# stevewongv/Sparse2Dense

Measured on AMD Instinct MI355X. Metric: LiDAR frames/sec (fwd+bwd), 150k-pt 0.1m-voxel synthetic Waymo scene, higher is better.
Workload: dtype bf16 (sparse stack: bf16 storage; dense neck/head: bf16 NHWC activations; fp32 accumulate, statistics, master weights, optimizer)

## Files before the change

### include/s2d.h

```cpp
#ifndef S2D_H_
#define S2D_H_

#include <stddef.h>
#include <stdint.h>

#ifdef __cplusplus
extern "C" {
#endif

typedef void *s2d_stream_t;

#define S2D_OK 0
#define S2D_ERR_INVALID_ARG (-1)
#define S2D_ERR_UNSUPPORTED (-2)
#define S2D_ERR_CAPACITY (-3)
#define S2D_ERR_WORKSPACE (-4)
#define S2D_ERR_COMM (-5)

int s2d_version(void);
int s2d_last_error(char *buf, size_t buf_len);
int s2d_build_info(char *buf, size_t buf_len);

size_t s2d_voxelize_batch_workspace_bytes(int frames, const int64_t *point_offsets, int max_points, int max_voxels);
int s2d_voxelize_batch_run(const float *points, int frames, const int64_t *point_offsets, int ndim,
                           const float coors_range[6], const float voxel_size[3], int max_points, int max_voxels,
                           float *voxels, int32_t *coors4, int32_t *num_points, float *mean, int32_t *out_m,
                           int32_t *out_base, void *ws, size_t ws_bytes, s2d_stream_t stream);
size_t s2d_voxelize_workspace_bytes(int64_t n_points, int max_points, int max_voxels);
int s2d_voxelize_run(const float *points, int64_t n_points, int ndim, const float coors_range[6],
                     const float voxel_size[3], int max_points, int max_voxels, float *voxels,
                     int32_t *coors, int32_t *num_points, float *mean, int32_t *out_m, void *ws,
                     size_t ws_bytes, s2d_stream_t stream);

size_t s2d_rulebook_workspace_bytes(int batch, const int32_t shape[3], int64_t n_rows);

int s2d_rulebook_subm_build(const int32_t *coors, int64_t n, int batch, const int32_t shape[3],
                            const int32_t ksize[3], const int32_t dilation[3], int32_t *nbr_out,
                            int32_t *pair_count, void *ws, size_t ws_bytes, s2d_stream_t stream);

int s2d_rulebook_conv_count(const int32_t *coors, int64_t n, int batch, const int32_t shape[3],
                            const int32_t ksize[3], const int32_t stride[3],
                            const int32_t padding[3], const int32_t dilation[3], int32_t *out_n,
                            void *ws, size_t ws_bytes, s2d_stream_t stream);
int s2d_rulebook_conv_fill(const int32_t *coors, int64_t n, int batch, const int32_t shape[3],
                           const int32_t ksize[3], const int32_t stride[3],
                           const int32_t padding[3], const int32_t dilation[3], int64_t n_out,
                           int32_t *out_coors, int32_t *nbr_out, int32_t *nbr_in,
                           int32_t *pair_count, void *ws, size_t ws_bytes, s2d_stream_t stream);

int s2d_rulebook_chain_supported(int batch, const int32_t shape0[3], int n_strided, const int32_t *ksize,
                                 const int32_t *stride, const int32_t *padding);
size_t s2d_rulebook_chain_workspace_bytes(int batch, const int32_t shape0[3], int n_strided, const int32_t *ksize,
                                          const int32_t *stride, const int32_t *padding);
int s2d_rulebook_chain_plan(const int32_t *coors0, int64_t n0, int batch, const int32_t shape0[3], int n_strided,
                            const int32_t *ksize, const int32_t *stride, const int32_t *padding, int32_t *counts,
                            void *ws, size_t ws_bytes, s2d_stream_t stream);
int s2d_rulebook_chain_fill(const int32_t *coors0, int64_t n0, int batch, const int32_t shape0[3], int n_strided,
                            const int32_t *ksize, const int32_t *stride, const int32_t *padding, const int64_t *n_rows,
                            int32_t *const *out_coors, int32_t *const *subm_nbr, int32_t *const *conv_nbr_out,
                            int32_t *const *conv_nbr_in, int32_t *pair_counts, int32_t *child, void *ws, size_t ws_bytes,
                            s2d_stream_t stream);

int s2d_spconv_fwd_f32(const float *in_feat, int64_t n_in, const float *weight, const float *bias,
                       const int32_t *nbr, int64_t n_out, int kvol, int cin, int cout,
                       float *out_feat, s2d_stream_t stream);
int s2d_spconv_bf16_supported(int cin, int cout);
int s2d_spconv_pack_weights_bf16(const float *weight, int kvol, int cin, int cout, int transpose,
                                 int flip, void *packed, s2d_stream_t stream);
int s2d_spconv_fwd_bf16(const float *in_feat, int64_t n_in, const void *packed_weight,
                        const float *bias, const int32_t *nbr, int64_t n_out, int kvol, int cin,
                        int cout, float *out_feat, s2d_stream_t stream);
size_t s2d_spconv_wgrad_workspace_bytes(int64_t n_out, int kvol, int cin, int cout);
int s2d_spconv_wgrad_f32(const float *in_feat, int64_t n_in, const float *dout, const int32_t *nbr,
                         int64_t n_out, int kvol, int cin, int cout, float *dweight, void *ws,
                         size_t ws_bytes, s2d_stream_t stream);

int s2d_spconv_wgrad_bf16(const float *in_feat, int64_t n_in, const float *dout, const int32_t *nbr,
                          int64_t n_out, int kvol, int cin, int cout, float *dweight, void *ws,
                          size_t ws_bytes, s2d_stream_t stream);

size_t s2d_bn1d_workspace_bytes(int64_t n, int c);
int s2d_bn1d_stats_f32(const float *x, int64_t n, int c, float *stats, void *ws, size_t ws_bytes,
                       s2d_stream_t stream);
int s2d_bn1d_finalize_fwd_f32(const float *stats, const float *count, const float *gamma,
                              const float *beta, float eps, float momentum, int c, float *mean,
                              float *invstd, float *scale, float *shift, float *running_mean,
                              float *running_var, int64_t *batches_tracked, s2d_stream_t stream);
int s2d_bn1d_finalize_bwd_f32(const float *sums_local, const float *sums_global, const float *count,
                              const float *gamma, const float *mean, const float *invstd, int c,
                              float *dgamma, float *dbeta, float *a, float *b, float *d,
                              s2d_stream_t stream);
int s2d_bn1d_stats_finalize_f32(const float *x, int64_t n, int c, const float *gamma,
                                const float *beta, float eps, float momentum, float *mean,
                                float *invstd, float *scale, float *shift, float *running_mean,
                                float *running_var, int64_t *batches_tracked, void *ws,
                                size_t ws_bytes, s2d_stream_t stream);
int s2d_bn1d_bwd_reduce_finalize_f32(const float *dy, const float *y, const float *x, int relu,
                                     int64_t n, int c, const float *gamma, const float *mean,
                                     const float *invstd, float *g_out, float *dgamma, float *dbeta,
                                     float *a, float *b, float *d, void *ws, size_t ws_bytes,
                                     s2d_stream_t stream);
int s2d_bn1d_apply_f32(const float *x, const float *scale, const float *shift,
                       const float *residual, int relu, int64_t n, int c, float *y,
                       s2d_stream_t stream);
int s2d_bn1d_bwd_reduce_f32(const float *dy, const float *y, const float *x, int relu, int64_t n,
                            int c, float *g_out, float *sums, void *ws, size_t ws_bytes,
                            s2d_stream_t stream);
int s2d_bn1d_bwd_apply_f32(const float *g, const float *x, const float *a, const float *b,
                           const float *d, int64_t n, int c, float *dx, s2d_stream_t stream);

// ... 424 lines not shown
```

### sparse2dense_amd/_lib.py

```python
import ctypes
import os

_HERE = os.path.dirname(os.path.abspath(__file__))
LIB_PATH = os.path.join(_HERE, "lib", "libs2d_hip.so")

c_i32p = ctypes.c_void_p
c_f32p = ctypes.c_void_p
_I3 = ctypes.c_int32 * 3
_PFN_GEO = [ctypes.c_int64, ctypes.c_int, ctypes.c_int, ctypes.c_float, ctypes.c_float, ctypes.c_float, ctypes.c_float]
_F3 = ctypes.c_float * 3
_F6 = ctypes.c_float * 6

SIGNATURES = {
    "s2d_version": (ctypes.c_int, []),
    "s2d_last_error": (ctypes.c_int, [ctypes.c_char_p, ctypes.c_size_t]),
    "s2d_build_info": (ctypes.c_int, [ctypes.c_char_p, ctypes.c_size_t]),
    "s2d_debug_lds_fill": (ctypes.c_int, [ctypes.c_float, ctypes.c_int, ctypes.c_int, ctypes.c_void_p, ctypes.c_void_p]),
    "s2d_voxelize_workspace_bytes": (ctypes.c_size_t, [ctypes.c_int64, ctypes.c_int, ctypes.c_int]),
    "s2d_voxelize_run": (ctypes.c_int, [c_f32p, ctypes.c_int64, ctypes.c_int, _F6, _F3, ctypes.c_int, ctypes.c_int,
                                        c_f32p, c_i32p, c_i32p, c_f32p, c_i32p, ctypes.c_void_p, ctypes.c_size_t,
                                        ctypes.c_void_p]),
    "s2d_voxelize_batch_workspace_bytes": (ctypes.c_size_t, [ctypes.c_int, ctypes.c_void_p, ctypes.c_int, ctypes.c_int]),
    "s2d_voxelize_batch_run": (ctypes.c_int, [c_f32p, ctypes.c_int, ctypes.c_void_p, ctypes.c_int, _F6, _F3, ctypes.c_int, ctypes.c_int,
                                              c_f32p, c_i32p, c_i32p, c_f32p, c_i32p, c_i32p, ctypes.c_void_p, ctypes.c_size_t, ctypes.c_void_p]),
    "s2d_rulebook_workspace_bytes": (ctypes.c_size_t, [ctypes.c_int, _I3, ctypes.c_int64]),
    "s2d_rulebook_subm_build": (ctypes.c_int, [c_i32p, ctypes.c_int64, ctypes.c_int, _I3, _I3, _I3, c_i32p, c_i32p,
                                               ctypes.c_void_p, ctypes.c_size_t, ctypes.c_void_p]),
    "s2d_rulebook_conv_count": (ctypes.c_int, [c_i32p, ctypes.c_int64, ctypes.c_int, _I3, _I3, _I3, _I3, _I3, c_i32p,
                                               ctypes.c_void_p, ctypes.c_size_t, ctypes.c_void_p]),
    "s2d_rulebook_conv_fill": (ctypes.c_int, [c_i32p, ctypes.c_int64, ctypes.c_int, _I3, _I3, _I3, _I3, _I3,
                                              ctypes.c_int64, c_i32p, c_i32p, c_i32p, c_i32p, ctypes.c_void_p,
                                              ctypes.c_size_t, ctypes.c_void_p]),
    "s2d_conv2d_pack_batch_bf16": (ctypes.c_int, [ctypes.c_int] + [ctypes.c_void_p] * 9),
    "s2d_pfn_supported": (ctypes.c_int, [ctypes.c_int] * 4),
    "s2d_pfn_blocks": (ctypes.c_int, [ctypes.c_int64]),
    "s2d_pfn_bwd_cols": (ctypes.c_int, []),
    "s2d_pfn_stats_f32": (ctypes.c_int, [c_f32p, c_i32p, c_i32p, c_f32p, ctypes.c_int64, ctypes.c_int, ctypes.c_int, ctypes.c_float, ctypes.c_float,
                                         ctypes.c_float, ctypes.c_float, c_f32p, ctypes.c_void_p]),
    "s2d_pfn_apply_max_f32": (ctypes.c_int, [c_f32p, c_i32p, c_i32p, c_f32p, c_f32p, c_f32p, ctypes.c_int64, ctypes.c_int, ctypes.c_int, ctypes.c_float,
                                             ctypes.c_float, ctypes.c_float, ctypes.c_float, c_f32p, ctypes.c_void_p, ctypes.c_void_p]),
    "s2d_pfn_bwd_f32": (ctypes.c_int, [c_f32p, c_i32p, c_i32p, c_f32p, c_f32p, ctypes.c_void_p, ctypes.c_int64, ctypes.c_int, ctypes.c_int, ctypes.c_float,
                                       ctypes.c_float, ctypes.c_float, ctypes.c_float, c_f32p, ctypes.c_void_p]),
    "s2d_pfn2_supported": (ctypes.c_int, [ctypes.c_int] * 5),
    "s2d_pfn2_bwd_rows": (ctypes.c_int, []),
    "s2d_pfn2_bwd_cols": (ctypes.c_int, []),
    "s2d_pfn2_stats1_f32": (ctypes.c_int, [c_f32p, c_i32p, c_i32p, c_f32p] + _PFN_GEO + [c_f32p, ctypes.c_void_p]),
    "s2d_pfn2_stats2_f32": (ctypes.c_int, [c_f32p, c_i32p, c_i32p, c_f32p, c_f32p, c_f32p] + _PFN_GEO + [c_f32p, ctypes.c_void_p]),
    "s2d_pfn2_apply_max_f32": (ctypes.c_int, [c_f32p, c_i32p, c_i32p, c_f32p, c_f32p, c_f32p, c_f32p] + _PFN_GEO
                               + [c_f32p, ctypes.c_void_p, c_f32p, ctypes.c_void_p]),
    "s2d_pfn2_bwd_f32": (ctypes.c_int, [c_f32p, c_i32p, c_i32p, c_f32p, c_f32p, c_f32p, c_f32p, c_f32p, ctypes.c_void_p] + _PFN_GEO
                         + [c_f32p, ctypes.c_void_p]),
    "s2d_rulebook_chain_supported": (ctypes.c_int, [ctypes.c_int, _I3, ctypes.c_int, ctypes.c_void_p, ctypes.c_void_p, ctypes.c_void_p]),
    "s2d_rulebook_chain_workspace_bytes": (ctypes.c_size_t, [ctypes.c_int, _I3, ctypes.c_int, ctypes.c_void_p, ctypes.c_void_p,
                                                             ctypes.c_void_p]),
    "s2d_rulebook_chain_plan": (ctypes.c_int, [c_i32p, ctypes.c_int64, ctypes.c_int, _I3, ctypes.c_int, ctypes.c_void_p, ctypes.c_void_p,
                                               ctypes.c_void_p, c_i32p, ctypes.c_void_p, ctypes.c_size_t, ctypes.c_void_p]),
    "s2d_rulebook_chain_fill": (ctypes.c_int, [c_i32p, ctypes.c_int64, ctypes.c_int, _I3, ctypes.c_int, ctypes.c_void_p, ctypes.c_void_p,
                                               ctypes.c_void_p, ctypes.c_void_p, ctypes.c_void_p, ctypes.c_void_p, ctypes.c_void_p,
                                               ctypes.c_void_p, c_i32p, c_i32p, ctypes.c_void_p, ctypes.c_size_t, ctypes.c_void_p]),
    "s2d_spconv_fwd_f32": (ctypes.c_int, [c_f32p, ctypes.c_int64, c_f32p, c_f32p, c_i32p, ctypes.c_int64, ctypes.c_int,
                                          ctypes.c_int, ctypes.c_int, c_f32p, ctypes.c_void_p]),
    "s2d_spconv_bf16_supported": (ctypes.c_int, [ctypes.c_int, ctypes.c_int]),
    "s2d_spconv_pack_weights_bf16": (ctypes.c_int, [c_f32p, ctypes.c_int, ctypes.c_int, ctypes.c_int, ctypes.c_int,
                                                    ctypes.c_int, ctypes.c_void_p, ctypes.c_void_p]),
    "s2d_spconv_fwd_bf16": (ctypes.c_int, [c_f32p, ctypes.c_int64, ctypes.c_void_p, c_f32p, c_i32p, ctypes.c_int64,
                                           ctypes.c_int, ctypes.c_int, ctypes.c_int, c_f32p, ctypes.c_void_p]),
    "s2d_spconv_wgrad_workspace_bytes": (ctypes.c_size_t, [ctypes.c_int64, ctypes.c_int, ctypes.c_int, ctypes.c_int]),
    "s2d_spconv_wgrad_f32": (ctypes.c_int, [c_f32p, ctypes.c_int64, c_f32p, c_i32p, ctypes.c_int64, ctypes.c_int,
                                            ctypes.c_int, ctypes.c_int, c_f32p, ctypes.c_void_p, ctypes.c_size_t,
                                            ctypes.c_void_p]),
    "s2d_spconv_wgrad_bf16": (ctypes.c_int, [c_f32p, ctypes.c_int64, c_f32p, c_i32p, ctypes.c_int64, ctypes.c_int,
                                             ctypes.c_int, ctypes.c_int, c_f32p, ctypes.c_void_p, ctypes.c_size_t,
                                             ctypes.c_void_p]),
    "s2d_bn1d_workspace_bytes": (ctypes.c_size_t, [ctypes.c_int64, ctypes.c_int]),
    "s2d_bn1d_stats_f32": (ctypes.c_int, [c_f32p, ctypes.c_int64, ctypes.c_int, c_f32p, ctypes.c_void_p,
                                          ctypes.c_size_t, ctypes.c_void_p]),
    "s2d_bn1d_finalize_fwd_f32": (ctypes.c_int, [c_f32p, c_f32p, c_f32p, c_f32p, ctypes.c_float, ctypes.c_float, ctypes.c_int,
                                                 c_f32p, c_f32p, c_f32p, c_f32p, c_f32p, c_f32p, ctypes.c_void_p,
                                                 ctypes.c_void_p]),
    "s2d_bn1d_finalize_bwd_f32": (ctypes.c_int, [c_f32p, c_f32p, c_f32p, c_f32p, c_f32p, c_f32p, ctypes.c_int, c_f32p,
                                                 c_f32p, c_f32p, c_f32p, c_f32p, ctypes.c_void_p]),
    "s2d_bn1d_stats_finalize_f32": (ctypes.c_int, [c_f32p, ctypes.c_int64, ctypes.c_int, c_f32p, c_f32p, ctypes.c_float,
                                                   ctypes.c_float, c_f32p, c_f32p, c_f32p, c_f32p, c_f32p, c_f32p,
                                                   ctypes.c_void_p, ctypes.c_void_p, ctypes.c_size_t, ctypes.c_void_p]),
    "s2d_bn1d_bwd_reduce_finalize_f32": (ctypes.c_int, [c_f32p, c_f32p, c_f32p, ctypes.c_int, ctypes.c_int64, ctypes.c_int,
                                                        c_f32p, c_f32p, c_f32p, c_f32p, c_f32p, c_f32p, c_f32p, c_f32p,
                                                        c_f32p, ctypes.c_void_p, ctypes.c_size_t, ctypes.c_void_p]),
    "s2d_bn1d_apply_f32": (ctypes.c_int, [c_f32p, c_f32p, c_f32p, c_f32p, ctypes.c_int, ctypes.c_int64, ctypes.c_int,
                                          c_f32p, ctypes.c_void_p]),
    "s2d_bn1d_bwd_reduce_f32": (ctypes.c_int, [c_f32p, c_f32p, c_f32p, ctypes.c_int, ctypes.c_int64, ctypes.c_int,
                                               c_f32p, c_f32p, ctypes.c_void_p, ctypes.c_size_t, ctypes.c_void_p]),
    "s2d_bn1d_bwd_apply_f32": (ctypes.c_int, [c_f32p, c_f32p, c_f32p, c_f32p, c_f32p, ctypes.c_int64, ctypes.c_int,
                                              c_f32p, ctypes.c_void_p]),
    "s2d_pointwise_conv_f32": (ctypes.c_int, [c_f32p, c_f32p, c_f32p, ctypes.c_int, ctypes.c_int, ctypes.c_int,
                                              ctypes.c_int64, c_f32p, ctypes.c_void_p]),
    "s2d_comm_load_library": (ctypes.c_int, [ctypes.c_char_p]),
    "s2d_comm_available": (ctypes.c_int, []),
    "s2d_comm_unique_id": (ctypes.c_int, [ctypes.c_void_p]),
    "s2d_comm_init": (ctypes.c_int, [ctypes.c_void_p, ctypes.c_int, ctypes.c_int]),
    "s2d_comm_ranks": (ctypes.c_int, []),
    "s2d_comm_shutdown": (ctypes.c_int, []),
    "s2d_convt3d_mfma_supported": (ctypes.c_int, [ctypes.c_int, ctypes.c_int]),
    "s2d_convt3d_mfma_packed_elems": (ctypes.c_size_t, [ctypes.c_int, ctypes.c_int]),
    "s2d_convt3d_mfma_pack_weights": (ctypes.c_int, [c_f32p, ctypes.c_int, ctypes.c_int, ctypes.c_void_p, ctypes.c_void_p]),
    "s2d_convt3d_mfma_fwd": (ctypes.c_int, [c_f32p, ctypes.c_void_p, c_f32p] + [ctypes.c_int] * 6 + [c_f32p, ctypes.c_void_p]),
    "s2d_convt3d_mfma_stats_tiles": (ctypes.c_int64, [ctypes.c_int] * 5),
    "s2d_convt3d_mfma_fwd_stats": (ctypes.c_int, [c_f32p, ctypes.c_void_p, c_f32p] + [ctypes.c_int] * 6 + [c_f32p, c_f32p, ctypes.c_void_p]),
# ... 343 lines not shown
```

### sparse2dense_amd/csrc/voxelize.hip

```cpp
#include <limits.h>

#include "s2d_common.h"
#include "scan.h"

namespace s2d {

constexpr uint32_t VOX_EMPTY = 0x7F7F7F7Fu;
constexpr int IDX_EMPTY = 0x7F7F7F7F;

struct VoxParams {
    float lo[3];
    float vs[3];
    int grid[3];
    int ndim;
    int max_points;
    int max_voxels;
    uint32_t table_mask;
    int table_shift;
};

__device__ __forceinline__ uint32_t vox_hash(uint32_t key, int shift) { return (key * 2654435761u) >> shift; }

__device__ __forceinline__ uint32_t vox_table_insert(uint32_t *__restrict__ keys, int *__restrict__ first, uint32_t key, uint32_t h, uint32_t mask, int i) {
    while (true) {
// ... 545 lines not shown
}

extern "C" size_t s2d_voxelize_batch_workspace_bytes(int frames, const int64_t *point_offsets, int max_points, int max_voxels) {
    if (frames <= 0 || frames > VOXB_MAX_FRAMES || !point_offsets || max_points <= 0 || max_voxels <= 0) return 0;
    return voxb_carve(nullptr, frames, point_offsets, max_points, max_voxels).bytes;
}

extern "C" int s2d_voxelize_batch_run(const float *points, int frames, const int64_t *point_offsets, int ndim, const float coors_range[6],
                                      const float voxel_size[3], int max_points, int max_voxels, float *voxels, int32_t *coors4,
                                      int32_t *num_points, float *mean, int32_t *out_m, int32_t *out_base, void *ws, size_t ws_bytes,
                                      s2d_stream_t stream) {
    S2D_CHECK_ARG(frames > 0 && frames <= VOXB_MAX_FRAMES && point_offsets, "voxelize_batch: 1..%d frames", VOXB_MAX_FRAMES);
    S2D_CHECK_ARG(ndim >= 3 && max_points > 0 && max_voxels > 0, "voxelize_batch: bad ndim/max_points/max_voxels");
    S2D_CHECK_ARG(coors_range && voxel_size && out_m && out_base && coors4 && voxels && num_points, "voxelize_batch: null argument");
    const int64_t n_points = point_offsets[frames];
    S2D_CHECK_ARG(point_offsets[0] == 0 && n_points >= 0 && n_points < (int64_t)INT_MAX / 2, "voxelize_batch: bad offsets");
    S2D_CHECK_ARG(n_points == 0 || points, "voxelize_batch: null points");
    hipStream_t st = (hipStream_t)stream;
    VoxParams p;
    double cells = 1.0;
    for (int j = 0; j < 3; ++j) {
        p.lo[j] = coors_range[j];
        p.vs[j] = voxel_size[j];
        float g = (coors_range[3 + j] - coors_range[j]) / voxel_size[j];
        p.grid[j] = (int)nearbyintf(g);
        S2D_CHECK_ARG(p.grid[j] > 0, "voxelize_batch: empty grid on axis %d", j);
        cells *= p.grid[j];
    }
    if (cells >= (double)VOX_EMPTY) {
        set_error("voxelize_batch: grid of %.0f cells exceeds the key space", cells);
        return S2D_ERR_UNSUPPORTED;
    }
    p.ndim = ndim; p.max_points = max_points; p.max_voxels = max_voxels; p.table_mask = 0; p.table_shift = 0;
    VoxbWs w = voxb_carve(ws, frames, point_offsets, max_points, max_voxels);
    if (ws_bytes < w.bytes || !ws) {
        set_error("voxelize_batch: workspace too small (%zu < %zu)", ws_bytes, w.bytes);
        return S2D_ERR_WORKSPACE;
    }
    VoxBatch vb;
    vb.frames = frames;
    int64_t rows = 0;
    size_t tb = 0;
    for (int b = 0; b < frames; ++b) {
        S2D_CHECK_ARG(point_offsets[b + 1] >= point_offsets[b], "voxelize_batch: offsets must not decrease");
        const int64_t nb = point_offsets[b + 1] - point_offsets[b];
        const size_t t = voxb_table(nb);
        int lg = 0;
        while (((size_t)1 << lg) < t) ++lg;
        vb.offs[b] = (int)point_offsets[b];
        vb.table_base[b] = (int)tb;
        vb.table_mask[b] = (uint32_t)(t - 1);
        vb.table_shift[b] = 32 - lg;
        tb += t;
        rows += nb < max_voxels ? nb : max_voxels;
    }
    vb.offs[frames] = (int)n_points;
    if (n_points == 0) {
        S2D_HIP(hipMemsetAsync(out_m, 0, sizeof(int32_t) * frames, st));
        S2D_HIP(hipMemsetAsync(out_base, 0, sizeof(int32_t) * (frames + 1), st));
        return S2D_OK;
    }
    const int n = (int)n_points;
    S2D_HIP(hipMemsetAsync(w.keys, 0x7F, w.clear_bytes, st));
    const dim3 blk(256);
    hipLaunchKernelGGL(voxb_insert_kernel, dim3((n + 255) / 256), blk, 0, st, points, n, p, vb, w.keys, w.first, w.pt_slot, w.total + 1);
    S2D_LAUNCH_CHECK();
    FirstFlagIn fin{w.pt_slot, w.first};
    VoxbRankOut fout{w.pt_slot, w.rank_of_slot, w.frame_start_rank, vb, n};
    int rc = device_exclusive_scan_onepass(fin, fout, n_points, w.flags, w.total, w.total + 1, st);
    if (rc) return rc;
    hipLaunchKernelGGL(voxb_frame_counts_kernel, dim3(1), dim3(64), 0, st, w.frame_start_rank, vb, max_voxels, out_m, w.out_base, out_base, w.total + 1);
    hipLaunchKernelGGL(voxb_assign_kernel, dim3((n + 255) / 256), blk, 0, st, w.pt_slot, w.first, w.keys, w.rank_of_slot, w.frame_start_rank,
                       w.out_base, n, p, vb, w.vid, coors4);
    rc = vox_select_launch(w.pt_slot, w.first, w.vid, n, max_points, rows, w.ksmall, w.sel, st);
    if (rc) return rc;
    hipLaunchKernelGGL(voxb_fill_kernel, dim3((unsigned)ceil_div(rows * max_points, 256)), blk, 0, st, points, w.ksmall, w.out_base, frames, ndim,
                       max_points, voxels, num_points);
    if (mean)
        hipLaunchKernelGGL(voxb_mean_kernel, dim3((unsigned)ceil_div(rows * ndim, 256)), blk, 0, st, points, w.ksmall, w.out_base, frames, ndim,
                           max_points, mean);
    S2D_LAUNCH_CHECK();
    return S2D_OK;
}
```

### sparse2dense_amd/hip_ops.py

```python
import ctypes
import os
from dataclasses import dataclass
from typing import Optional, Tuple

import numpy as np
import torch

from . import _lib
from ._lib import check, f3, f6, i3


def _stream():
    return torch._C._cuda_getCurrentRawStream(torch.cuda.current_device())


def _ptr(t: Optional[torch.Tensor]):
    if t is None:
        return None
    return t.data_ptr()


def _need_gpu(*ts):
    for t in ts:
        if t is not None and not t.is_cuda:
            raise _lib.S2DError("sparse2dense_amd HIP op called with a CPU tensor: there is no CPU fallback")


def _ws(nbytes, device):
    return torch.empty(max(int(nbytes), 256), dtype=torch.uint8, device=device)


def _ws_shared(nbytes, device):
    from .dense2d import _ws as shared_ws
    return shared_ws(nbytes, device)


def voxelize_async(points: torch.Tensor, voxel_size, coors_range, max_points: int, max_voxels: int, with_mean=True):
    lib = _lib.load()
    _need_gpu(points)
    points = points.contiguous().float()
    n, ndim = points.shape
    dev = points.device
    rows = max(min(n, max_voxels), 1)
    voxels = torch.empty((rows, max_points, ndim), dtype=torch.float32, device=dev)
    coors = torch.empty((rows, 3), dtype=torch.int32, device=dev)
    num = torch.empty((rows,), dtype=torch.int32, device=dev)
    mean = torch.empty((rows, ndim), dtype=torch.float32, device=dev) if with_mean else None
    out_m = torch.zeros((1,), dtype=torch.int32, device=dev)
    ws = _ws(lib.s2d_voxelize_workspace_bytes(n, max_points, max_voxels), dev)
    check(lib.s2d_voxelize_run(_ptr(points), n, ndim, f6(coors_range), f3(voxel_size), max_points, max_voxels,
                               _ptr(voxels), _ptr(coors), _ptr(num), _ptr(mean), _ptr(out_m), _ptr(ws), ws.numel(),
                               _stream()), "s2d_voxelize_run")
    return voxels, coors, num, mean, out_m


def voxelize(points: torch.Tensor, voxel_size, coors_range, max_points: int, max_voxels: int, with_mean=True):
    voxels, coors, num, mean, out_m = voxelize_async(points, voxel_size, coors_range, max_points, max_voxels, with_mean)
    m = int(out_m.item())
    if m < 0:
        raise _lib.S2DError("s2d_voxelize_run: the look-back scan timed out on the device (csrc/scan.h); no voxels were produced")
    return voxels[:m], coors[:m], num[:m], (mean[:m] if with_mean else None)


def voxelize_batch_launch(points_cat: torch.Tensor, offsets, voxel_size, coors_range, max_points: int, max_voxels: int):
    lib = _lib.load()
    _need_gpu(points_cat)
    points_cat = points_cat.contiguous().float()
    n, ndim = points_cat.shape
    frames = len(offsets) - 1
    assert offsets[0] == 0 and offsets[-1] == n
    offs = (ctypes.c_int64 * (frames + 1))(*[int(o) for o in offsets])
    dev = points_cat.device
    rows = max(sum(min(int(offsets[b + 1] - offsets[b]), max_voxels) for b in range(frames)), 1)
    voxels = torch.empty((rows, max_points, ndim), dtype=torch.float32, device=dev)
    coors = torch.empty((rows, 4), dtype=torch.int32, device=dev)
    num = torch.empty((rows,), dtype=torch.int32, device=dev)
    mean = torch.empty((rows, ndim), dtype=torch.float32, device=dev)
    out_m = torch.empty((frames,), dtype=torch.int32, device=dev)
    out_base = torch.empty((frames + 1,), dtype=torch.int32, device=dev)
    ws = _ws(lib.s2d_voxelize_batch_workspace_bytes(frames, offs, max_points, max_voxels), dev)
    rec = None
    if PROFILE is not None:
        rec = dict(kernel="voxelize", tag="voxelize", cin=0, cout=0, n_points=int(n), frames=frames, out_base=out_base, max_points=max_points,
                   ndim=int(ndim), start=torch.cuda.Event(enable_timing=True), end=torch.cuda.Event(enable_timing=True))
        rec["start"].record()
    check(lib.s2d_voxelize_batch_run(_ptr(points_cat), frames, offs, ndim, f6(coors_range), f3(voxel_size), max_points, max_voxels,
                                     _ptr(voxels), _ptr(coors), _ptr(num), _ptr(mean), _ptr(out_m), _ptr(out_base), _ptr(ws), ws.numel(),
                                     _stream()), "s2d_voxelize_batch_run")
    if rec is not None:
        rec["end"].record()
        PROFILE.append(rec)
    return (voxels, coors, num, mean, out_base)


def voxelize_batch_collect(pending, base):
    voxels, coors, num, mean, out_base = pending
    m = int(base[-1])
    if m < 0:
        raise _lib.S2DError("s2d_voxelize_batch_run: the look-back scan timed out on the device (csrc/scan.h); no voxels were produced")
    counts = torch.tensor([int(base[b + 1]) - int(base[b]) for b in range(len(base) - 1)], dtype=torch.int64, device=voxels.device)
    return voxels[:m], coors[:m], num[:m], mean[:m], counts


def voxelize_batch(points_cat: torch.Tensor, offsets, voxel_size, coors_range, max_points: int, max_voxels: int):
    pending = voxelize_batch_launch(points_cat, offsets, voxel_size, coors_range, max_points, max_voxels)
    return voxelize_batch_collect(pending, pending[4].cpu().tolist())


@dataclass
class Rulebook:
    subm: bool
    kvol: int
    n_in: int
    n_out: int
    nbr_out: torch.Tensor
    nbr_in: Optional[torch.Tensor]
    pair_count: torch.Tensor
    out_coors: Optional[torch.Tensor]
    out_shape: Tuple[int, int, int]
    coors: Optional[torch.Tensor] = None

    def pairs(self):
        nb = self.nbr_out.cpu().numpy()
        res = []
        for k in range(self.kvol):
            o = np.nonzero(nb[k] >= 0)[0]
            res.append((nb[k][o].astype(np.int64), o.astype(np.int64)))
        return res


def conv_out_shape(shape, ksize, stride, padding, dilation=(1, 1, 1)):
    return tuple((int(shape[i]) + 2 * padding[i] - dilation[i] * (ksize[i] - 1) - 1) // stride[i] + 1 for i in range(3))


def build_subm_rulebook(coors: torch.Tensor, batch: int, shape, ksize, dilation=(1, 1, 1)) -> Rulebook:
    lib = _lib.load()
    _need_gpu(coors)
    coors = coors.contiguous()
    assert coors.dtype == torch.int32 and coors.dim() == 2 and coors.shape[1] == 4
    n = coors.shape[0]
    dev = coors.device
    kvol = int(ksize[0] * ksize[1] * ksize[2])
    nbr = torch.empty((kvol, n), dtype=torch.int32, device=dev)
    cnt = torch.empty((kvol,), dtype=torch.int32, device=dev)
    ws = _ws(lib.s2d_rulebook_workspace_bytes(batch, i3(shape), n), dev)
    rec = None
    if PROFILE is not None:
        rec = dict(kernel="rulebook_subm", tag="rulebook", cin=0, cout=0, n_out=int(n), kvol=kvol, pairs=cnt,
                   start=torch.cuda.Event(enable_timing=True), end=torch.cuda.Event(enable_timing=True))
        rec["start"].record()
    check(lib.s2d_rulebook_subm_build(_ptr(coors), n, batch, i3(shape), i3(ksize), i3(dilation), _ptr(nbr), _ptr(cnt),
                                      _ptr(ws), ws.numel(), _stream()), "s2d_rulebook_subm_build")
    if rec is not None:
        rec["end"].record()
        PROFILE.append(rec)
    return Rulebook(True, kvol, n, n, nbr, None, cnt, None, tuple(int(s) for s in shape), coors=coors)


class ConvRulebookJob:

    def __init__(self, coors, batch, shape, ksize, stride, padding, dilation=(1, 1, 1)):
        self.lib = _lib.load()
        _need_gpu(coors)
        self.coors = coors.contiguous()
        assert self.coors.dtype == torch.int32 and self.coors.shape[1] == 4
        self.batch, self.shape = int(batch), tuple(int(s) for s in shape)
        self.ksize, self.stride = tuple(map(int, ksize)), tuple(map(int, stride))
        self.padding, self.dilation = tuple(map(int, padding)), tuple(map(int, dilation))
        self.out_shape = conv_out_shape(self.shape, self.ksize, self.stride, self.padding, self.dilation)
        self.kvol = self.ksize[0] * self.ksize[1] * self.ksize[2]
        dev = self.coors.device
        self.ws = _ws(self.lib.s2d_rulebook_workspace_bytes(self.batch, i3(self.out_shape), 0), dev)
        self.out_n = torch.zeros((1,), dtype=torch.int32, device=dev)

    def count(self):
        n = self.coors.shape[0]
        self._rec = None
        if PROFILE is not None:
            self._rec = dict(kernel="rulebook_conv", tag="rulebook", cin=0, cout=0, n_in=int(n), kvol=self.kvol,
                             start=torch.cuda.Event(enable_timing=True), end=torch.cuda.Event(enable_timing=True),
                             start2=torch.cuda.Event(enable_timing=True), end2=torch.cuda.Event(enable_timing=True))
            self._rec["start"].record()
        check(self.lib.s2d_rulebook_conv_count(_ptr(self.coors), n, self.batch, i3(self.shape), i3(self.ksize),
                                               i3(self.stride), i3(self.padding), i3(self.dilation), _ptr(self.out_n),
                                               _ptr(self.ws), self.ws.numel(), _stream()), "s2d_rulebook_conv_count")
        if self._rec is not None:
            self._rec["end"].record()
        return self

# ... 484 lines not shown
```

### sparse2dense_amd/voxel_ops.py

```python
import numpy as np
import torch

from . import hip_ops as H


def points_to_voxel(points, voxel_size, coors_range, max_points=35, reverse_index=True, max_voxels=20000,
                    return_mean=False):
    is_np = isinstance(points, np.ndarray)
    if is_np:
        if not torch.cuda.is_available():
            raise RuntimeError("points_to_voxel: no ROCm device visible and there is no CPU fallback")
        pts = torch.from_numpy(np.ascontiguousarray(points, dtype=np.float32)).cuda()
    else:
        pts = points
    vs = np.asarray(voxel_size, dtype=np.float32)
    rng = np.asarray(coors_range, dtype=np.float32)
    voxels, coors, num, mean = H.voxelize(pts, vs, rng, int(max_points), int(max_voxels), with_mean=return_mean)
    if not reverse_index:
        coors = coors.flip(1)
    if is_np:
        out = (voxels.cpu().numpy(), coors.cpu().numpy(), num.cpu().numpy())
        return out + (mean.cpu().numpy(),) if return_mean else out
    return (voxels, coors, num, mean) if return_mean else (voxels, coors, num)


class VoxelGenerator:
    def __init__(self, voxel_size, point_cloud_range, max_num_points, max_voxels=20000):
        point_cloud_range = np.array(point_cloud_range, dtype=np.float32)
        voxel_size = np.array(voxel_size, dtype=np.float32)
        grid_size = (point_cloud_range[3:] - point_cloud_range[:3]) / voxel_size
        self._grid_size = np.round(grid_size).astype(np.int64)
        self._voxel_size = voxel_size
        self._point_cloud_range = point_cloud_range
        self._max_num_points = max_num_points
        self._max_voxels = max_voxels

    def generate(self, points, max_voxels=-1, return_mean=False):
        if max_voxels == -1:
            max_voxels = self._max_voxels
        return points_to_voxel(points, self._voxel_size, self._point_cloud_range, self._max_num_points, True,
                               max_voxels, return_mean=return_mean)

    @property
    def voxel_size(self):
        return self._voxel_size

    @property
    def max_num_points_per_voxel(self):
        return self._max_num_points

    @property
    def point_cloud_range(self):
        return self._point_cloud_range

    @property
    def grid_size(self):
        return self._grid_size


def voxelize_batches(requests):
    pend = []
    for generator, point_clouds, prefix in requests:
        offs = [0]
        for pts in point_clouds:
            offs.append(offs[-1] + int(pts.shape[0]))
        cat = point_clouds[0] if len(point_clouds) == 1 else torch.cat([p.float() for p in point_clouds], 0)
        pend.append((prefix, H.voxelize_batch_launch(cat, offs, generator.voxel_size, generator.point_cloud_range,
                                                     generator.max_num_points_per_voxel, generator._max_voxels)))
    bases = torch.cat([p[1][4] for p in pend]).cpu().tolist()
    out, at = {}, 0
    for prefix, p in pend:
        k = p[4].numel()
        v, c, n, m, counts = H.voxelize_batch_collect(p, bases[at:at + k])
        at += k
        out.update({prefix + "voxels": v, prefix + "coordinates": c, prefix + "num_points": n, prefix + "num_voxels": counts,
                    prefix + "voxel_mean": m})
    return out


def voxelize_batch(generator: VoxelGenerator, point_clouds, max_voxels=-1, prefix="", batched=True):
    mv = generator._max_voxels if max_voxels == -1 else max_voxels
    if batched and point_clouds[0].is_cuda and len(point_clouds) <= 64:
        offs = [0]
        for pts in point_clouds:
            offs.append(offs[-1] + int(pts.shape[0]))
        cat = point_clouds[0] if len(point_clouds) == 1 else torch.cat([p.float() for p in point_clouds], 0)
        v, c, n, m, counts = H.voxelize_batch(cat, offs, generator.voxel_size, generator.point_cloud_range,
                                              generator.max_num_points_per_voxel, mv)
        return {prefix + "voxels": v, prefix + "coordinates": c, prefix + "num_points": n, prefix + "num_voxels": counts,
                prefix + "voxel_mean": m}
    pend = [H.voxelize_async(pts, generator.voxel_size, generator.point_cloud_range, generator.max_num_points_per_voxel,
                             generator._max_voxels if max_voxels == -1 else max_voxels, with_mean=True)
            for pts in point_clouds]
    counts = torch.cat([p[4] for p in pend]).cpu().tolist()
    if counts and min(counts) < 0:
        raise H._lib.S2DError("s2d_voxelize_run: the look-back scan timed out on the device (csrc/scan.h)")
    vs, cs, ns, ms = [], [], [], []
    for b, ((v, c, n, m, _), k) in enumerate(zip(pend, counts)):
        cb = torch.empty((k, 4), dtype=torch.int32, device=c.device)
        cb[:, 0] = b
        cb[:, 1:] = c[:k]
        vs.append(v[:k]); cs.append(cb); ns.append(n[:k]); ms.append(m[:k])
    dev = vs[0].device
    return {
        prefix + "voxels": torch.cat(vs, 0),
        prefix + "coordinates": torch.cat(cs, 0),
        prefix + "num_points": torch.cat(ns, 0),
        prefix + "num_voxels": torch.tensor(counts, dtype=torch.int64, device=dev),
        prefix + "voxel_mean": torch.cat(ms, 0),
    }
```

Baseline: 225.7.

## Voxelize all segments in one radix-sort based multi-segment launch

Measured after the change: 228.7 (median of 5 runs). 1.4% higher.

```diff
diff --git a/include/s2d.h b/include/s2d.h
--- a/include/s2d.h
+++ b/include/s2d.h
@@ -26,6 +26,21 @@
                            const float coors_range[6], const float voxel_size[3], int max_points, int max_voxels,
                            float *voxels, int32_t *coors4, int32_t *num_points, float *mean, int32_t *out_m,
                            int32_t *out_base, void *ws, size_t ws_bytes, s2d_stream_t stream);
+typedef struct s2d_vox_segment {
+    float coors_range[6];
+    float voxel_size[3];
+    int32_t max_points, max_voxels, ndim, frames;
+    const float *const *frame_points;
+    const int64_t *frame_counts;
+    float *voxels;
+    int32_t *coors4;
+    int32_t *num_points;
+    float *mean;
+    int32_t *out_m;
+} s2d_vox_segment;
+size_t s2d_voxelize_multi_workspace_bytes(int segments, const s2d_vox_segment *segs);
+int s2d_voxelize_multi_run(int segments, const s2d_vox_segment *segs, int32_t *out_base_all, void *ws, size_t ws_bytes,
+                           s2d_stream_t stream);
 size_t s2d_voxelize_workspace_bytes(int64_t n_points, int max_points, int max_voxels);
 int s2d_voxelize_run(const float *points, int64_t n_points, int ndim, const float coors_range[6],
                      const float voxel_size[3], int max_points, int max_voxels, float *voxels,
diff --git a/sparse2dense_amd/_lib.py b/sparse2dense_amd/_lib.py
--- a/sparse2dense_amd/_lib.py
+++ b/sparse2dense_amd/_lib.py
@@ -10,6 +10,15 @@
 _PFN_GEO = [ctypes.c_int64, ctypes.c_int, ctypes.c_int, ctypes.c_float, ctypes.c_float, ctypes.c_float, ctypes.c_float]
 _F3 = ctypes.c_float * 3
 _F6 = ctypes.c_float * 6
+
+
+
+class VoxSegment(ctypes.Structure):
+    _fields_ = [("coors_range", _F6), ("voxel_size", _F3), ("max_points", ctypes.c_int32), ("max_voxels", ctypes.c_int32),
+                ("ndim", ctypes.c_int32), ("frames", ctypes.c_int32), ("frame_points", ctypes.c_void_p), ("frame_counts", ctypes.c_void_p),
+                ("voxels", ctypes.c_void_p), ("coors4", ctypes.c_void_p), ("num_points", ctypes.c_void_p), ("mean", ctypes.c_void_p),
+                ("out_m", ctypes.c_void_p)]
+
 
 SIGNATURES = {
     "s2d_version": (ctypes.c_int, []),
@@ -23,6 +32,8 @@
     "s2d_voxelize_batch_workspace_bytes": (ctypes.c_size_t, [ctypes.c_int, ctypes.c_void_p, ctypes.c_int, ctypes.c_int]),
     "s2d_voxelize_batch_run": (ctypes.c_int, [c_f32p, ctypes.c_int, ctypes.c_void_p, ctypes.c_int, _F6, _F3, ctypes.c_int, ctypes.c_int,
                                               c_f32p, c_i32p, c_i32p, c_f32p, c_i32p, c_i32p, ctypes.c_void_p, ctypes.c_size_t, ctypes.c_void_p]),
+    "s2d_voxelize_multi_workspace_bytes": (ctypes.c_size_t, [ctypes.c_int, ctypes.c_void_p]),
+    "s2d_voxelize_multi_run": (ctypes.c_int, [ctypes.c_int, ctypes.c_void_p, c_i32p, ctypes.c_void_p, ctypes.c_size_t, ctypes.c_void_p]),
     "s2d_rulebook_workspace_bytes": (ctypes.c_size_t, [ctypes.c_int, _I3, ctypes.c_int64]),
     "s2d_rulebook_subm_build": (ctypes.c_int, [c_i32p, ctypes.c_int64, ctypes.c_int, _I3, _I3, _I3, c_i32p, c_i32p,
                                                ctypes.c_void_p, ctypes.c_size_t, ctypes.c_void_p]),
diff --git a/sparse2dense_amd/csrc/voxelize.hip b/sparse2dense_amd/csrc/voxelize.hip
--- a/sparse2dense_amd/csrc/voxelize.hip
+++ b/sparse2dense_amd/csrc/voxelize.hip
@@ -651,3 +651,345 @@
     S2D_LAUNCH_CHECK();
     return S2D_OK;
 }
+
+#include <rocprim/device/device_radix_sort.hpp>
+
+namespace s2d {
+
+constexpr int VM_MAX_SEGMENTS = 8;
+constexpr int VM_MAX_ENTRIES = VM_MAX_SEGMENTS * VOXB_MAX_FRAMES;
+constexpr int VM_CELL_BITS = 27;
+constexpr int VM_IDX_BITS = 28;
+constexpr uint64_t VM_IDX_MASK = ((uint64_t)1 << VM_IDX_BITS) - 1;
+
+struct VmSeg {
+    float lo[3], vs[3];
+    int grid[3];
+    int ndim, max_points, max_voxels;
+    int first_entry, frames;
+    int base_off;
+    float *voxels;
+    int32_t *coors4, *num_points;
+    float *mean;
+    int32_t *out_m;
+};
+struct VmEntry {
+    const float *points;
+    int start;
+    int seg;
+};
+struct VmBlob {
+    uint32_t w[512];
+};
+constexpr int VM_BLOB_WORDS = 512;
+
+__global__ __launch_bounds__(VM_BLOB_WORDS) void vm_init_kernel(VmBlob blob, int word0, int words, uint32_t *__restrict__ tables,
+                                                                unsigned long long *__restrict__ granules, int n_granules, int *__restrict__ total) {
+    const int t = threadIdx.x;
+    if (t < words) tables[word0 + t] = blob.w[t];
+    if (word0 == 0) {
+        for (int i = t; i < n_granules; i += VM_BLOB_WORDS) granules[i] = 0ull;
+        if (t < 2) total[t] = 0;
+    }
+}
+
+__device__ __forceinline__ int vm_find_entry(const VmEntry *__restrict__ ent, int entries, int g) {
+    int lo = 0, hi = entries - 1;
+    while (lo < hi) {
+        const int mid = (lo + hi + 1) >> 1;
+        if (ent[mid].start <= g) lo = mid; else hi = mid - 1;
+    }
+    return lo;
+}
+
+__global__ __launch_bounds__(256) void vm_key_kernel(const VmSeg *__restrict__ segs, const VmEntry *__restrict__ ent, int entries, int n, int cell_bits,
+                                                     uint64_t sentinel, uint64_t *__restrict__ keys) {
+    const int g = blockIdx.x * 256 + threadIdx.x;
+    int e = vm_find_entry(ent, entries, blockIdx.x * 256);
+    if (g >= n) return;
+    while (e + 1 < entries && g >= ent[e + 1].start) ++e;
+    const VmEntry en = ent[e];
+    const VmSeg &p = segs[en.seg];
+    const float *pt = en.points + (int64_t)(g - en.start) * p.ndim;
+    int c[3];
+    bool ok = true;
+#pragma unroll
+    for (int j = 0; j < 3; ++j) {
+        float q = __fdiv_rn(__fsub_rn(pt[j], p.lo[j]), p.vs[j]);
+        float f = floorf(q);
+        ok = ok && (f >= 0.0f) && (f < (float)p.grid[j]);
+        c[j] = (int)f;
+    }
+    uint64_t hi = sentinel;
+    if (ok) {
+        const uint32_t key = ((uint32_t)c[2] * (uint32_t)p.grid[1] + (uint32_t)c[1]) * (uint32_t)p.grid[0] + (uint32_t)c[0];
+        hi = ((uint64_t)e << cell_bits) | key;
+    }
+    keys[g] = (hi << VM_IDX_BITS) | (uint64_t)g;
+}
+
+__global__ __launch_bounds__(256) void vm_heads_kernel(const uint64_t *__restrict__ sorted, int n, uint64_t sentinel, uint8_t *__restrict__ flags) {
+    const int j = blockIdx.x * 256 + threadIdx.x;
+    if (j >= n) return;
+    const uint64_t k = sorted[j], hi = k >> VM_IDX_BITS;
+    const bool head = hi != sentinel && (j == 0 || (sorted[j - 1] >> VM_IDX_BITS) != hi);
+    flags[k & VM_IDX_MASK] = head ? 1 : 0;
+}
+
+struct VmFlagIn {
+    const uint8_t *flags;
+    __device__ int operator()(int64_t i) const { return flags[i]; }
+};
+struct VmRankOut {
+    int *rank;
+    __device__ void operator()(int64_t i, int, int run) const { rank[i] = run; }
+};
+
+__global__ __launch_bounds__(VM_MAX_ENTRIES) void vm_counts_kernel(const VmSeg *__restrict__ segs, int n_segs, const VmEntry *__restrict__ ent, int entries,
+                                                                   int n, const int *__restrict__ rank, const int *__restrict__ total,
+                                                                   int *__restrict__ start_rank, int *__restrict__ row_base,
+                                                                   int32_t *__restrict__ out_base_all) {
+    __shared__ int cnt[VM_MAX_ENTRIES];
+    __shared__ int seg_rows[VM_MAX_SEGMENTS];
+    const int e = threadIdx.x;
+    const bool err = total[1] == 1;
+    int m = 0, s = 0;
+    if (e < entries) {
+        s = ent[e].seg;
+        const int a = ent[e].start, b = e + 1 < entries ? ent[e + 1].start : n;
+        const int ra = a < n ? rank[a] : total[0], rb = b < n ? rank[b] : total[0];
+        m = rb - ra;
+        m = m < segs[s].max_voxels ? m : segs[s].max_voxels;
+        if (err) m = 0;
+        start_rank[e] = ra;
+        cnt[e] = m;
+    }
+    __syncthreads();
+    if (e < entries) {
+        const VmSeg &p = segs[s];
+        int base = 0;
+        for (int q = p.first_entry; q < e; ++q) base += cnt[q];
+        row_base[e] = base;
+        const int f = e - p.first_entry;
+        p.out_m[f] = m;
+        out_base_all[p.base_off + f] = base;
+        if (f == p.frames - 1) {
+            out_base_all[p.base_off + p.frames] = err ? -1 : base + m;
+            seg_rows[s] = base + m;
+        }
+    }
+    __syncthreads();
+    if (e == 0) {
+        int all = 0;
+        for (int q = 0; q < n_segs; ++q) all += seg_rows[q];
+        int words = 0;
+        for (int q = 0; q < n_segs; ++q) words += segs[q].frames + 1;
+        out_base_all[words] = err ? -1 : all;
+    }
+}
+
+__global__ __launch_bounds__(256) void vm_fill_kernel(const VmSeg *__restrict__ segs, const VmEntry *__restrict__ ent, const uint64_t *__restrict__ sorted,
+                                                      int n, int cell_bits, uint64_t sentinel, const int *__restrict__ rank,
+                                                      const int *__restrict__ start_rank, const int *__restrict__ row_base,
+                                                      const int *__restrict__ total) {
+    const int j = blockIdx.x * 256 + threadIdx.x;
+    if (j >= n || total[1] == 1) return;
+    const uint64_t k = sorted[j], hi = k >> VM_IDX_BITS;
+    if (hi == sentinel) return;
+    const int e = (int)(hi >> cell_bits);
+    const VmEntry en = ent[e];
+    const VmSeg &p = segs[en.seg];
+    const int P = p.max_points, ndim = p.ndim;
+    int r = 0;
+    while (r < P && j - r - 1 >= 0 && (sorted[j - r - 1] >> VM_IDX_BITS) == hi) ++r;
+    if (r >= P) return;
+    const int head = (int)(sorted[j - r] & VM_IDX_MASK);
+    const int local = rank[head] - start_rank[e];
+    if (local >= p.max_voxels) return;
+    const int64_t row = (int64_t)row_base[e] + local;
+    const float *src = en.points + (int64_t)((int)(k & VM_IDX_MASK) - en.start) * ndim;
+    float *dst = p.voxels + (row * P + r) * ndim;
+    for (int c = 0; c < ndim; ++c) dst[c] = src[c];
+    if (r != 0) return;
+    int cnt = 1;
+    while (cnt < P && j + cnt < n && (sorted[j + cnt] >> VM_IDX_BITS) == hi) ++cnt;
+    for (int q = cnt * ndim; q < P * ndim; ++q) dst[q] = 0.0f;
+    p.num_points[row] = cnt;
+    uint32_t key = (uint32_t)(hi & (((uint64_t)1 << cell_bits) - 1));
+    const int x = key % (uint32_t)p.grid[0];
+    key /= (uint32_t)p.grid[0];
+    const int y = key % (uint32_t)p.grid[1];
+    const int z = key / (uint32_t)p.grid[1];
+    reinterpret_cast<int4 *>(p.coors4)[row] = int4{e - p.first_entry, z, y, x};
+    if (!p.mean) return;
+    for (int c = 0; c < ndim; ++c) {
+        float s = 0.0f;
+        for (int q = 0; q < cnt; ++q)
+            s = __fadd_rn(s, en.points[(int64_t)((int)(sorted[j + q] & VM_IDX_MASK) - en.start) * ndim + c]);
+        p.mean[row * ndim + c] = __fdiv_rn(s, (float)cnt);
+    }
+}
+
+struct VmPlan {
+    int n_segs, entries, n, cell_bits, table_words;
+    VmSeg segs[VM_MAX_SEGMENTS];
+    VmEntry ent[VM_MAX_ENTRIES];
+};
+struct VmWs {
+    uint32_t *tables;
+    uint64_t *keys_a, *keys_b;
+    uint8_t *flags;
+    int *rank, *total, *start_rank, *row_base;
+    unsigned long long *granules;
+    char *sort_tmp;
+    size_t sort_bytes, bytes;
+};
+
+static int vm_plan(int n_segs, const s2d_vox_segment *sg, VmPlan &pl) {
+    S2D_CHECK_ARG(n_segs >= 1 && n_segs <= VM_MAX_SEGMENTS && sg, "voxelize_multi: 1..%d segments", VM_MAX_SEGMENTS);
+    memset(&pl, 0, sizeof(pl));
+    pl.n_segs = n_segs;
+    int64_t n = 0;
+    double max_cells = 1.0;
+    int base_off = 0;
+    for (int s = 0; s < n_segs; ++s) {
+        const s2d_vox_segment &g = sg[s];
+        VmSeg &p = pl.segs[s];
+        S2D_CHECK_ARG(g.frames >= 1 && g.frames <= VOXB_MAX_FRAMES && g.frame_points && g.frame_counts, "voxelize_multi: segment %d: 1..%d frames",
+                      s, VOXB_MAX_FRAMES);
+        S2D_CHECK_ARG(g.ndim >= 3 && g.max_points > 0 && g.max_voxels > 0, "voxelize_multi: segment %d: bad ndim/max_points/max_voxels", s);
+        double cells = 1.0;
+        for (int j = 0; j < 3; ++j) {
+            p.lo[j] = g.coors_range[j];
+            p.vs[j] = g.voxel_size[j];
+            float gr = (g.coors_range[3 + j] - g.coors_range[j]) / g.voxel_size[j];
+            S2D_CHECK_ARG(gr >= 0.5f && gr < 2147483520.0f, "voxelize_multi: segment %d: empty or unbounded grid on axis %d", s, j);
+            p.grid[j] = (int)nearbyintf(gr);
+            S2D_CHECK_ARG(p.grid[j] > 0, "voxelize_multi: segment %d: empty grid on axis %d", s, j);
+            cells *= p.grid[j];
+        }
+        max_cells = cells > max_cells ? cells : max_cells;
+        p.ndim = g.ndim; p.max_points = g.max_points; p.max_voxels = g.max_voxels;
+        p.first_entry = pl.entries; p.frames = g.frames; p.base_off = base_off;
+        p.voxels = g.voxels; p.coors4 = g.coors4; p.num_points = g.num_points; p.mean = g.mean; p.out_m = g.out_m;
+        base_off += g.frames + 1;
+        for (int f = 0; f < g.frames; ++f) {
+            S2D_CHECK_ARG(g.frame_counts[f] >= 0, "voxelize_multi: segment %d frame %d: negative point count", s, f);
+            S2D_CHECK_ARG(g.frame_counts[f] == 0 || g.frame_points[f], "voxelize_multi: segment %d frame %d: null points", s, f);
+            if (n + g.frame_counts[f] >= ((int64_t)1 << VM_IDX_BITS)) {
+                set_error("voxelize_multi: more than 2^%d - 1 points in one chain", VM_IDX_BITS);
+                return S2D_ERR_UNSUPPORTED;
+            }
+            VmEntry &en = pl.ent[pl.entries++];
+            en.points = g.frame_points[f]; en.start = (int)n; en.seg = s;
+            n += g.frame_counts[f];
+        }
+    }
+    if (max_cells > (double)(((uint64_t)1 << VM_CELL_BITS) - 1)) {
+        set_error("voxelize_multi: grid of %.0f cells exceeds the %d key bits", max_cells, VM_CELL_BITS);
+        return S2D_ERR_UNSUPPORTED;
+    }
+    pl.n = (int)n;
+    pl.cell_bits = 1;
+    while ((double)(((uint64_t)1 << pl.cell_bits) - 1) < max_cells) ++pl.cell_bits;
+    pl.table_words = (int)((sizeof(VmSeg) * VM_MAX_SEGMENTS + sizeof(VmEntry) * pl.entries) / 4);
+    return S2D_OK;
+}
+
+static int vm_entry_bits(const VmPlan &pl) {
+    int b = 0;
+    while ((1 << b) < pl.entries) ++b;
+    return b;
+}
+
+static int vm_sort(void *tmp, size_t &bytes, rocprim::double_buffer<uint64_t> &keys, const VmPlan &pl, hipStream_t st) {
+    S2D_HIP(rocprim::radix_sort_keys(tmp, bytes, keys, (unsigned)pl.n, (unsigned)VM_IDX_BITS, (unsigned)(VM_IDX_BITS + pl.cell_bits + vm_entry_bits(pl)), st));
+    return S2D_OK;
+}
+
+static int vm_carve(void *ws, const VmPlan &pl, VmWs &w) {
+    const size_t n = (size_t)(pl.n > 0 ? pl.n : 1);
+    Carver c(ws);
+    w.tables = c.take<uint32_t>((sizeof(VmSeg) * VM_MAX_SEGMENTS + sizeof(VmEntry) * VM_MAX_ENTRIES) / 4);
+    w.keys_a = c.take<uint64_t>(n);
+    w.keys_b = c.take<uint64_t>(n);
+    w.flags = c.take<uint8_t>(n);
+    w.rank = c.take<int>(n);
+    w.granules = c.take<unsigned long long>(scan1_num_blocks(pl.n));
+    w.total = c.take<int>(2);
+    w.start_rank = c.take<int>(VM_MAX_ENTRIES);
+    w.row_base = c.take<int>(VM_MAX_ENTRIES);
+    w.sort_bytes = 0;
+    if (pl.n > 0) {
+        rocprim::double_buffer<uint64_t> keys(w.keys_a, w.keys_b);
+        int rc = vm_sort(nullptr, w.sort_bytes, keys, pl, (hipStream_t)0);
+        if (rc) return rc;
+    }
+    w.sort_tmp = c.take<char>(w.sort_bytes > 0 ? w.sort_bytes : 1);
+    w.bytes = c.total();
+    return S2D_OK;
+}
+
+}
+
+extern "C" size_t s2d_voxelize_multi_workspace_bytes(int segments, const s2d_vox_segment *segs) {
+    static thread_local VmPlan pl;
+    VmWs w;
+    if (vm_plan(segments, segs, pl) != S2D_OK || vm_carve(nullptr, pl, w) != S2D_OK) return 0;
+    return w.bytes;
+}
+
+extern "C" int s2d_voxelize_multi_run(int segments, const s2d_vox_segment *segs, int32_t *out_base_all, void *ws, size_t ws_bytes, s2d_stream_t stream) {
+    static thread_local VmPlan pl;
+    int rc = vm_plan(segments, segs, pl);
+    if (rc) return rc;
+    S2D_CHECK_ARG(out_base_all, "voxelize_multi: null out_base_all");
+    for (int s = 0; s < segments; ++s)
+        S2D_CHECK_ARG(segs[s].voxels && segs[s].coors4 && segs[s].num_points && segs[s].out_m, "voxelize_multi: segment %d: null output", s);
+    VmWs w;
+    rc = vm_carve(ws, pl, w);
+    if (rc) return rc;
+    if (ws_bytes < w.bytes || !ws) {
+        set_error("voxelize_multi: workspace too small (%zu < %zu)", ws_bytes, w.bytes);
+        return S2D_ERR_WORKSPACE;
+    }
+    hipStream_t st = (hipStream_t)stream;
+    const int n = pl.n;
+    static thread_local uint32_t host[(sizeof(VmSeg) * VM_MAX_SEGMENTS + sizeof(VmEntry) * VM_MAX_ENTRIES) / 4];
+    memcpy(host, pl.segs, sizeof(VmSeg) * VM_MAX_SEGMENTS);
+    memcpy(host + sizeof(VmSeg) * VM_MAX_SEGMENTS / 4, pl.ent, sizeof(VmEntry) * pl.entries);
+    const VmSeg *d_segs = reinterpret_cast<const VmSeg *>(w.tables);
+    const VmEntry *d_ent = reinterpret_cast<const VmEntry *>(w.tables + sizeof(VmSeg) * VM_MAX_SEGMENTS / 4);
+    for (int w0 = 0; w0 < pl.table_words; w0 += VM_BLOB_WORDS) {
+        VmBlob blob;
+        const int words = pl.table_words - w0 < VM_BLOB_WORDS ? pl.table_words - w0 : VM_BLOB_WORDS;
+        memcpy(blob.w, host + w0, (size_t)words * 4);
+        hipLaunchKernelGGL(vm_init_kernel, dim3(1), dim3(VM_BLOB_WORDS), 0, st, blob, w0, words, w.tables, w.granules, scan1_num_blocks(n), w.total);
+    }
+    S2D_LAUNCH_CHECK();
+    const uint64_t *sorted = w.keys_a;
+    const uint64_t sentinel = ((uint64_t)1 << (64 - VM_IDX_BITS)) - 1;
+    const dim3 blk(256), grid((unsigned)ceil_div(n, 256));
+    if (n > 0) {
+        hipLaunchKernelGGL(vm_key_kernel, grid, blk, 0, st, d_segs, d_ent, pl.entries, n, pl.cell_bits, sentinel, w.keys_a);
+        S2D_LAUNCH_CHECK();
+        rocprim::double_buffer<uint64_t> keys(w.keys_a, w.keys_b);
+        size_t sort_bytes = w.sort_bytes;
+        rc = vm_sort(w.sort_tmp, sort_bytes, keys, pl, st);
+        if (rc) return rc;
+        sorted = keys.current();
+        hipLaunchKernelGGL(vm_heads_kernel, grid, blk, 0, st, sorted, n, sentinel, w.flags);
+        S2D_LAUNCH_CHECK();
+        VmFlagIn fin{w.flags};
+        VmRankOut fout{w.rank};
+        rc = device_exclusive_scan_onepass(fin, fout, (int64_t)n, w.granules, w.total, w.total + 1, st);
+        if (rc) return rc;
+    }
+    hipLaunchKernelGGL(vm_counts_kernel, dim3(1), dim3(VM_MAX_ENTRIES), 0, st, d_segs, pl.n_segs, d_ent, pl.entries, n, w.rank, w.total, w.start_rank,
+                       w.row_base, out_base_all);
+    if (n > 0)
+        hipLaunchKernelGGL(vm_fill_kernel, grid, blk, 0, st, d_segs, d_ent, sorted, n, pl.cell_bits, sentinel, w.rank, w.start_rank, w.row_base,
+                           w.total);
+    S2D_LAUNCH_CHECK();
+    return S2D_OK;
+}
diff --git a/sparse2dense_amd/hip_ops.py b/sparse2dense_amd/hip_ops.py
--- a/sparse2dense_amd/hip_ops.py
+++ b/sparse2dense_amd/hip_ops.py
@@ -105,6 +105,65 @@
 def voxelize_batch(points_cat: torch.Tensor, offsets, voxel_size, coors_range, max_points: int, max_voxels: int):
     pending = voxelize_batch_launch(points_cat, offsets, voxel_size, coors_range, max_points, max_voxels)
     return voxelize_batch_collect(pending, pending[4].cpu().tolist())
+
+
+VOXELIZE_MULTI_MAX_SEGMENTS = 8
+
+
+def voxelize_multi_launch(segments):
+    lib = _lib.load()
+    n_seg = len(segments)
+    if not 1 <= n_seg <= VOXELIZE_MULTI_MAX_SEGMENTS:
+        raise _lib.S2DError(f"voxelize_multi_launch: 1..{VOXELIZE_MULTI_MAX_SEGMENTS} segments, got {n_seg}")
+    segs = (_lib.VoxSegment * n_seg)()
+    keep, outs = [], []
+    n_total = 0
+    dev = segments[0][0][0].device
+    words = sum(len(sg[0]) + 1 for sg in segments) + 1
+    out_base_all = torch.empty((words,), dtype=torch.int32, device=dev)
+    at = 0
+    for s, (clouds, voxel_size, coors_range, max_points, max_voxels) in enumerate(segments):
+        _need_gpu(*clouds)
+        clouds = [p.contiguous().float() for p in clouds]
+        frames = len(clouds)
+        ndim = int(clouds[0].shape[1])
+        counts = [int(p.shape[0]) for p in clouds]
+        if any(p.dim() != 2 or int(p.shape[1]) != ndim for p in clouds):
+            raise _lib.S2DError("voxelize_multi_launch: the frames of a segment must be [n, ndim] with one ndim")
+        ptrs = (ctypes.c_void_p * frames)(*[p.data_ptr() for p in clouds])
+        cnts = (ctypes.c_int64 * frames)(*counts)
+        rows = max(sum(min(c, max_voxels) for c in counts), 1)
+        voxels = torch.empty((rows, max_points, ndim), dtype=torch.float32, device=dev)
+        coors = torch.empty((rows, 4), dtype=torch.int32, device=dev)
+        num = torch.empty((rows,), dtype=torch.int32, device=dev)
+        mean = torch.empty((rows, ndim), dtype=torch.float32, device=dev)
+        out_m = torch.empty((frames,), dtype=torch.int32, device=dev)
+        g = segs[s]
+        g.coors_range, g.voxel_size = f6(coors_range), f3(voxel_size)
+        g.max_points, g.max_voxels, g.ndim, g.frames = int(max_points), int(max_voxels), ndim, frames
+        g.frame_points, g.frame_counts = ctypes.addressof(ptrs), ctypes.addressof(cnts)
+        g.voxels, g.coors4, g.num_points, g.mean, g.out_m = _ptr(voxels), _ptr(coors), _ptr(num), _ptr(mean), _ptr(out_m)
+        keep += [clouds, ptrs, cnts, out_m]
+        outs.append((voxels, coors, num, mean, out_base_all[at:at + frames + 1]))
+        at += frames + 1
+        n_total += sum(counts)
+    segs_p = ctypes.addressof(segs)
+    nbytes = lib.s2d_voxelize_multi_workspace_bytes(n_seg, segs_p)
+    if nbytes == 0:
+        raise _lib.S2DError(f"s2d_voxelize_multi_workspace_bytes: {_lib.last_error()}")
+    ws = _ws(nbytes, dev)
+    rec = None
+    if PROFILE is not None:
+        rec = dict(kernel="voxelize", tag="voxelize", cin=0, cout=0, n_points=int(n_total), frames=sum(len(sg[0]) for sg in segments),
+                   segments=n_seg, out_base=out_base_all, max_points=int(segments[0][3]), ndim=int(segs[0].ndim),
+                   start=torch.cuda.Event(enable_timing=True), end=torch.cuda.Event(enable_timing=True))
+        rec["start"].record()
+    check(lib.s2d_voxelize_multi_run(n_seg, segs_p, _ptr(out_base_all), _ptr(ws), ws.numel(), _stream()), "s2d_voxelize_multi_run")
+    if rec is not None:
+        rec["end"].record()
+        PROFILE.append(rec)
+    del keep
+    return outs, out_base_all
 
 
 @dataclass
diff --git a/sparse2dense_amd/voxel_ops.py b/sparse2dense_amd/voxel_ops.py
--- a/sparse2dense_amd/voxel_ops.py
+++ b/sparse2dense_amd/voxel_ops.py
@@ -59,15 +59,14 @@
 
 
 def voxelize_batches(requests):
-    pend = []
-    for generator, point_clouds, prefix in requests:
-        offs = [0]
-        for pts in point_clouds:
-            offs.append(offs[-1] + int(pts.shape[0]))
-        cat = point_clouds[0] if len(point_clouds) == 1 else torch.cat([p.float() for p in point_clouds], 0)
-        pend.append((prefix, H.voxelize_batch_launch(cat, offs, generator.voxel_size, generator.point_cloud_range,
-                                                     generator.max_num_points_per_voxel, generator._max_voxels)))
-    bases = torch.cat([p[1][4] for p in pend]).cpu().tolist()
+    pend, alls = [], []
+    step = H.VOXELIZE_MULTI_MAX_SEGMENTS
+    for i in range(0, len(requests), step):
+        outs, base_all = H.voxelize_multi_launch([(pc, g.voxel_size, g.point_cloud_range, g.max_num_points_per_voxel, g._max_voxels)
+                                                  for g, pc, _ in requests[i:i + step]])
+        pend += [(prefix, o) for (_, _, prefix), o in zip(requests[i:i + step], outs)]
+        alls.append(base_all[:-1])
+    bases = (alls[0] if len(alls) == 1 else torch.cat(alls)).cpu().tolist()
     out, at = {}, 0
     for prefix, p in pend:
         k = p[4].numel()
```
